# InterlinkLabs/e2e-tts

Measured on AMD Instinct MI355X. Metric: audio samples/sec (22.05 kHz, batch-32 per GPU, FastSpeech2 + HiFi-GAN inference, ids on host -> int16 PCM on host), higher is better.
Workload: dtype f32; 1 GPU; B=32/GPU fixed-length L=128 phonemes x 6 frames = T=768 frames (196608 samples, 8.92 s) per utterance; default model_config (6+6 FFT blocks H=384, HiFi-GAN V1), random-init weights; ids of tests/golden/bench_b32.npz (reference-pinned); global_batch=32, parallelism=utterance-sharded x1

## Files before the change

e2e_tts_amd/csrc/resblock_pair.hip:

```cpp
#include <algorithm>
#include <type_traits>

#include "kernels.h"

namespace e2etts {

typedef float f32x16 __attribute__((ext_vector_type(16)));
typedef __bf16 bf16x8 __attribute__((ext_vector_type(8)));
typedef __bf16 bf16x2 __attribute__((ext_vector_type(2)));

namespace {

constexpr int LDK = 36;
constexpr int MAX_HALO1 = 64;
constexpr size_t PAIR_MAX_LDS = 160 * 1024;

__device__ __forceinline__ unsigned pack_bf16(float a, float b) {
  const bf16x2 r = {(__bf16)a, (__bf16)b};
  return __builtin_bit_cast(unsigned, r);
}
__device__ __forceinline__ void split4(const float4 v, uint2& hi, uint2& lo) {
  hi.x = pack_bf16(v.x, v.y);
  hi.y = pack_bf16(v.z, v.w);
  const float hx = __builtin_bit_cast(float, hi.x << 16), hy = __builtin_bit_cast(float, hi.x & 0xffff0000u);
  const float hz = __builtin_bit_cast(float, hi.y << 16), hw = __builtin_bit_cast(float, hi.y & 0xffff0000u);
  lo.x = pack_bf16(v.x - hx, v.y - hy);
  lo.y = pack_bf16(v.z - hz, v.w - hw);
}

template <int BMI, int C, int WM, int WN>
constexpr int pair_threads() { return 64 * (BMI / WM) * (C / WN); }

template <int BMI, int C, int WM, int WN, int MODE, bool ACCUM>
__global__ __launch_bounds__((pair_threads<BMI, C, WM, WN>()), C == 32 ? 3 : 2) void resblock_pair_kernel(const PairParams p, const RowMap rm) {
  constexpr bool X3 = MODE != 0;
  constexpr bool SPLIT = MODE == 1;
  constexpr int KS = X3 ? 2 : 4;
  constexpr int NCH = C / 32;
  constexpr int NWN = C / WN;
  constexpr int MT = WM / 32, NT = WN / 32;
  constexpr int NWAVE = (BMI / WM) * NWN;
  static_assert(NWAVE == 4 || NWAVE == 8, "4 or 8 wavefronts per workgroup");
  constexpr int SROWS = NWAVE * 8;
  constexpr int AROWS = (BMI + MAX_HALO1 + SROWS - 1) / SROWS;

  extern __shared__ __attribute__((aligned(16))) float smem[];
  const int KW = p.KW, dil = p.dil;
  const int halo1 = dil * (KW - 1), pad1 = halo1 / 2, pad2 = (KW - 1) / 2;
  const int BMO = BMI - (KW - 1);
  const int irows = BMI + KW - 1;

  const int tid = threadIdx.x;
  const int lane = tid & 63, wave = __builtin_amdgcn_readfirstlane(tid >> 6);
  const int wm = wave / NWN, wn = wave % NWN;
  const int li = lane & 31, lh = lane >> 5;
  const int lrow = tid >> 3, lc4 = (tid & 7) * 4;

  int b, xb;
  if (rm.n > 0) {
    if (!rowmap_find(rm, (int)blockIdx.x, b, xb)) return;
  } else {
    b = blockIdx.y;
    xb = blockIdx.x;
  }
  const int t_act = p.act_rows ? min(p.act_rows[b], p.T) : p.T;
  const int mtiles = (t_act + BMO - 1) / BMO;
  const int eighth = (mtiles + 7) >> 3;
  const int tile = (xb & 7) * eighth + (xb >> 3);
  if ((xb >> 3) >= eighth || tile >= mtiles) return;

  const float* x_b = p.x + (long long)b * p.x_bs;
  float* out_b = p.out + (long long)b * p.out_bs;
  const __amdgpu_buffer_rsrc_t x_rsrc =
      __builtin_amdgcn_make_buffer_rsrc(const_cast<float*>(x_b), 0, (int)((long long)p.T * C * 4), 0x00020000);
  const int frag_words = NCH * KW * NCH * 1024;
  const __amdgpu_buffer_rsrc_t wf_rsrc =
      __builtin_amdgcn_make_buffer_rsrc(const_cast<float*>(p.wfrag), 0, 2 * frag_words * 4, 0x00020000);

  f32x16 acc[MT][NT];
#pragma unroll
  for (int m = 0; m < MT; ++m)
#pragma unroll
    for (int n = 0; n < NT; ++n)
#pragma unroll
      for (int r = 0; r < 16; ++r) acc[m][n][r] = 0.f;

  float4 areg[AROWS];
  bool aok[AROWS];
  const int srows = BMI + halo1;
  auto load_a = [&](int tile, int chunk) {
    const int x0 = tile * BMO - pad2 - pad1;
#pragma unroll
    for (int i = 0; i < AROWS; ++i) {
      const int r = lrow + i * SROWS;
      const int g = x0 + r;
      aok[i] = r < srows && g >= 0 && g < p.T;
      const int gc = min(max(g, 0), p.T - 1);
      areg[i] = __builtin_bit_cast(
          float4, __builtin_amdgcn_raw_buffer_load_b128(x_rsrc, (gc * C + lc4) * 4, chunk * 128, 0));
    }
  };
  auto store_a = [&]() {
#pragma unroll
    for (int i = 0; i < AROWS; ++i) {
      const int r = lrow + i * SROWS;
      if (r < srows) {
        float4 v = aok[i] ? areg[i] : make_float4(0.f, 0.f, 0.f, 0.f);
        v.x = fmaxf(v.x, v.x * p.slope); v.y = fmaxf(v.y, v.y * p.slope);
        v.z = fmaxf(v.z, v.z * p.slope); v.w = fmaxf(v.w, v.w * p.slope);
        if constexpr (X3) {
          uint2 hi, lo;
          split4(v, hi, lo);
          uint2* row = reinterpret_cast<uint2*>(smem + r * LDK);
          row[lc4 >> 2] = hi;
          row[8 + (lc4 >> 2)] = lo;
        } else {
          *reinterpret_cast<float4*>(smem + r * LDK + lc4) = v;
        }
      }
    }
  };

  constexpr bool DEEP = C == 32;
  float4 bfr[DEEP ? 2 : 1][KS][NT][SPLIT ? 2 : 1];
  auto load_frag_n = [&](auto par, int conv, int chunk, int j, int ks, int n) {
    constexpr int P = decltype(par)::value;
#pragma unroll
    for (int hl = 0; hl < (SPLIT ? 2 : 1); ++hl) {
      const int nt = wn * NT + n;
      const int piece = X3 ? ks * 2 + hl : ks;
      const int soff = (conv * frag_words + (((((nt * KW + j) * NCH + chunk) * 4) + piece) << 8)) * 4;
      bfr[P][ks][n][hl] = __builtin_bit_cast(float4, __builtin_amdgcn_raw_buffer_load_b128(wf_rsrc, lane * 16, soff, 0));
    }
  };
  auto load_frag = [&](int conv, int chunk, int j, int ks) {
#pragma unroll
    for (int n = 0; n < NT; ++n) load_frag_n(std::integral_constant<int, 0>{}, conv, chunk, j, ks, n);
  };
  auto mma_tap = [&](auto par, const float* a_base, int nconv, int nchunk, int nj) {
    constexpr int P = decltype(par)::value;
    if constexpr (DEEP) {
#pragma unroll
      for (int ks = 0; ks < KS; ++ks)
#pragma unroll
        for (int n = 0; n < NT; ++n) load_frag_n(std::integral_constant<int, 1 - P>{}, nconv, nchunk, nj, ks, n);
      __builtin_amdgcn_sched_barrier(0);
    }
#pragma unroll
    for (int ks = 0; ks < KS; ++ks) {
      if constexpr (X3) {
        bf16x8 ah[MT], al[MT];
#pragma unroll
        for (int m = 0; m < MT; ++m) {
          ah[m] = __builtin_bit_cast(bf16x8, *reinterpret_cast<const float4*>(a_base + m * 32 * LDK + ks * 8));
          if constexpr (SPLIT) al[m] = __builtin_bit_cast(bf16x8, *reinterpret_cast<const float4*>(a_base + m * 32 * LDK + 16 + ks * 8));
        }
#pragma unroll
        for (int n = 0; n < NT; ++n) {
#pragma unroll
          for (int m = 0; m < MT; ++m) {
            const bf16x8 bh = __builtin_bit_cast(bf16x8, bfr[P][ks][n][0]);
            if constexpr (SPLIT) {
              const bf16x8 bl = __builtin_bit_cast(bf16x8, bfr[P][ks][n][1]);
              acc[m][n] = __builtin_amdgcn_mfma_f32_32x32x16_bf16(bh, al[m], acc[m][n], 0, 0, 0);
              acc[m][n] = __builtin_amdgcn_mfma_f32_32x32x16_bf16(bl, ah[m], acc[m][n], 0, 0, 0);
            }
            acc[m][n] = __builtin_amdgcn_mfma_f32_32x32x16_bf16(bh, ah[m], acc[m][n], 0, 0, 0);
          }
          if constexpr (!DEEP) {
            __builtin_amdgcn_sched_barrier(0);
            load_frag_n(std::integral_constant<int, 0>{}, nconv, nchunk, nj, ks, n);
            __builtin_amdgcn_sched_barrier(0);
          }
        }
      } else {
        float4 af[MT];
#pragma unroll
        for (int m = 0; m < MT; ++m) af[m] = *reinterpret_cast<const float4*>(a_base + m * 32 * LDK + ks * 8);
#pragma unroll
        for (int n = 0; n < NT; ++n) {
          const float4 bf = bfr[P][ks][n][0];
#pragma unroll
          for (int m = 0; m < MT; ++m) {
            acc[m][n] = __builtin_amdgcn_mfma_f32_32x32x2f32(bf.x, af[m].x, acc[m][n], 0, 0, 0);
            acc[m][n] = __builtin_amdgcn_mfma_f32_32x32x2f32(bf.y, af[m].y, acc[m][n], 0, 0, 0);
            acc[m][n] = __builtin_amdgcn_mfma_f32_32x32x2f32(bf.z, af[m].z, acc[m][n], 0, 0, 0);
            acc[m][n] = __builtin_amdgcn_mfma_f32_32x32x2f32(bf.w, af[m].w, acc[m][n], 0, 0, 0);
          }
          if constexpr (!DEEP) {
            __builtin_amdgcn_sched_barrier(0);
            load_frag_n(std::integral_constant<int, 0>{}, nconv, nchunk, nj, ks, n);
            __builtin_amdgcn_sched_barrier(0);
          }
        }
      }
    }
  };
  auto run_taps = [&](auto par0, const float* a0, int row_step, int conv, int c, int nconv_end, int nchunk_end) {
    constexpr int P0 = DEEP ? decltype(par0)::value : 0;
    constexpr int P1 = DEEP ? 1 - P0 : 0;
    int j = 0;
    for (; j + 2 < KW; j += 2) {
      mma_tap(std::integral_constant<int, P0>{}, a0 + j * row_step, conv, c, j + 1);
      mma_tap(std::integral_constant<int, P1>{}, a0 + (j + 1) * row_step, conv, c, j + 2);
    }
    mma_tap(std::integral_constant<int, P0>{}, a0 + j * row_step, nconv_end, nchunk_end, 0);
  };

  auto epilogue1 = [&](int tile) {
    const int i0 = tile * BMO - pad2;
#pragma unroll
    for (int n = 0; n < NT; ++n) {
      const int chunk = wn * NT + n;
      float4 bq[4];
#pragma unroll
      for (int q = 0; q < 4; ++q) bq[q] = *reinterpret_cast<const float4*>(p.b1 + wn * WN + n * 32 + 8 * q + 4 * lh);
#pragma unroll
      for (int m = 0; m < MT; ++m) {
        const int row = wm * WM + m * 32 + li;
        const int g = i0 + row;
        const bool ok = g >= 0 && g < p.T;
        float* dst = smem + (chunk * irows + row) * LDK + 2 * lh;
#pragma unroll
        for (int q = 0; q < 4; ++q) {
          float v[4] = {acc[m][n][4 * q] + bq[q].x, acc[m][n][4 * q + 1] + bq[q].y, acc[m][n][4 * q + 2] + bq[q].z, acc[m][n][4 * q + 3] + bq[q].w};
#pragma unroll
          for (int i = 0; i < 4; ++i) {
            v[i] = fmaxf(v[i], v[i] * p.slope);
            v[i] = ok ? v[i] : 0.f;
            acc[m][n][4 * q + i] = 0.f;
          }
          if constexpr (!X3) {
            *reinterpret_cast<float4*>(smem + (chunk * irows + row) * LDK + 8 * q + 4 * lh) = make_float4(v[0], v[1], v[2], v[3]);
            continue;
          }
          uint2 hi;
          hi.x = pack_bf16(v[0], v[1]);
          hi.y = pack_bf16(v[2], v[3]);
          *reinterpret_cast<uint2*>(dst + 4 * q) = hi;
          if constexpr (SPLIT) {
            const float h0 = __builtin_bit_cast(float, hi.x << 16), h1 = __builtin_bit_cast(float, hi.x & 0xffff0000u);
            const float h2 = __builtin_bit_cast(float, hi.y << 16), h3 = __builtin_bit_cast(float, hi.y & 0xffff0000u);
            uint2 lo;
            lo.x = pack_bf16(v[0] - h0, v[1] - h1);
            lo.y = pack_bf16(v[2] - h2, v[3] - h3);
            *reinterpret_cast<uint2*>(dst + 16 + 4 * q) = lo;
          }
        }
      }
    }
  };

  constexpr int ELD = WN + 4;
  static_assert(NWAVE * 32 * ELD <= NCH * BMI * LDK, "epilogue patches must fit in the region (>= the intermediate: NCH x (BMI + KW - 1) rows)");
  constexpr int LPR = WN / 4, RPP = 64 / LPR, PASSES = 32 / RPP;
  const int prow = lane / LPR, pc4 = (lane % LPR) * 4;
  const int ecol = wn * WN + pc4;
  const float4 bias2 = *reinterpret_cast<const float4*>(p.b2 + ecol);
  auto epilogue2 = [&](int tile) {
    const int o0 = tile * BMO;
    const int t_end = min(o0 + BMO, p.T);
    float* patch = smem + wave * (32 * ELD);
#pragma unroll
    for (int m = 0; m < MT; ++m) {
      const int tb = o0 + wm * WM + m * 32;
      float4 resv[PASSES];
#pragma unroll
      for (int ps = 0; ps < PASSES; ++ps) {
        const int t = min(tb + ps * RPP + prow, p.T - 1);
        resv[ps] = *reinterpret_cast<const float4*>(x_b + (long long)t * C + ecol);
      }
      float4 accv[PASSES];
      if constexpr (ACCUM) {
#pragma unroll
        for (int ps = 0; ps < PASSES; ++ps) {
          const int t = min(tb + ps * RPP + prow, p.T - 1);
          accv[ps] = *reinterpret_cast<const float4*>(out_b + (long long)t * C + ecol);
        }
      }
#pragma unroll
      for (int n = 0; n < NT; ++n)
#pragma unroll
        for (int q = 0; q < 4; ++q)
          *reinterpret_cast<float4*>(patch + li * ELD + n * 32 + 8 * q + 4 * lh) =
              make_float4(acc[m][n][4 * q], acc[m][n][4 * q + 1], acc[m][n][4 * q + 2], acc[m][n][4 * q + 3]);
#pragma unroll
      for (int ps = 0; ps < PASSES; ++ps) {
        const int row = ps * RPP + prow;
        const int t = tb + row;
        float4 v = *reinterpret_cast<const float4*>(patch + row * ELD + pc4);
        v.x += bias2.x; v.y += bias2.y; v.z += bias2.z; v.w += bias2.w;
        const float4 rv = resv[ps];
        v.x += rv.x; v.y += rv.y; v.z += rv.z; v.w += rv.w;
        if constexpr (ACCUM) {
          const float4 ov = accv[ps];
          v.x += ov.x; v.y += ov.y; v.z += ov.z; v.w += ov.w;
          if (p.out_div != 1.0f) {
            v.x = v.x / p.out_div; v.y = v.y / p.out_div; v.z = v.z / p.out_div; v.w = v.w / p.out_div;
          }
        }
        if (t < t_end && wm * WM + m * 32 + row < BMO) {
          typedef float f32x4_t __attribute__((ext_vector_type(4)));
          const f32x4_t nv = {v.x, v.y, v.z, v.w};
          __builtin_nontemporal_store(nv, reinterpret_cast<f32x4_t*>(out_b + (long long)t * C + ecol));
        }
      }
    }
  };

  load_a(tile, 0);
  store_a();
#pragma unroll
  for (int ks = 0; ks < KS; ++ks) load_frag(0, 0, 0, ks);
  __builtin_amdgcn_s_waitcnt(0x0F70);

  for (int c = 0; c < NCH; ++c) {
    if (c + 1 < NCH) load_a(tile, c + 1);
    __syncthreads();
    const bool lastc = c + 1 == NCH;
    run_taps(std::integral_constant<int, 0>{}, smem + (wm * WM + li) * LDK + lh * 4, dil * LDK, 0, c, lastc ? 1 : 0, lastc ? 0 : c + 1);
    if (c + 1 < NCH) {
      __syncthreads();
      store_a();
    }
  }
  __syncthreads();
  epilogue1(tile);
  __syncthreads();
  for (int c = 0; c < NCH; ++c) {
    const bool lastc = c + 1 == NCH;
    run_taps(std::integral_constant<int, 1>{}, smem + (c * irows + wm * WM + li) * LDK + lh * 4, LDK, 1, c, 1, lastc ? 0 : c + 1);
  }
  __syncthreads();
  epilogue2(tile);
}

template <int BMI, int C, int WM, int WN, int MODE>
const char* launch_pair_cfg(const PairParams& p, hipStream_t s) {
  const int halo1 = p.dil * (p.KW - 1);
  const int BMO = BMI - (p.KW - 1);
  const size_t words = (size_t)std::max((BMI + halo1) * LDK, (C / 32) * (BMI + p.KW - 1) * LDK);
  const size_t lds = words * sizeof(float);
  if (lds > PAIR_MAX_LDS) return "resblock_pair: LDS region exceeds the CU's 160 KiB";
  const int mtiles = (p.T + BMO - 1) / BMO;
  dim3 grid((mtiles + 7) / 8 * 8, p.B);
  RowMap rm;
  if (p.act_rows && p.act_rows_host && p.B <= ROWMAP_MAX) {
    rm.n = p.B;
    rm.identity();
    rm.cum[0] = 0;
    for (int b = 0; b < p.B; ++b) {
      const int mt = (std::min(std::max(p.act_rows_host[b], 0), p.T) + BMO - 1) / BMO;
      rm.cum[b + 1] = rm.cum[b] + (mt + 7) / 8 * 8;
    }
    if (rm.cum[p.B] == 0) return nullptr;
    grid = dim3(rm.cum[p.B]);
  }
  constexpr int NTHR = pair_threads<BMI, C, WM, WN>();
  if (p.accumulate)
    hipLaunchKernelGGL((resblock_pair_kernel<BMI, C, WM, WN, MODE, true>), grid, dim3(NTHR), lds, s, p, rm);
  else
    hipLaunchKernelGGL((resblock_pair_kernel<BMI, C, WM, WN, MODE, false>), grid, dim3(NTHR), lds, s, p, rm);
  return hipGetLastError() == hipSuccess ? nullptr : "resblock_pair: launch failed";
}

template <int BMI, int C, int WM, int WN>
const char* launch_pair_mode(const PairParams& p, hipStream_t s) {
  static bool attr_done = false;
  if (!attr_done) {
    const int cap = C == 256 ? (int)PAIR_MAX_LDS : 80 * 1024;
    (void)hipFuncSetAttribute(reinterpret_cast<const void*>(&resblock_pair_kernel<BMI, C, WM, WN, 0, true>), hipFuncAttributeMaxDynamicSharedMemorySize, cap);
    (void)hipFuncSetAttribute(reinterpret_cast<const void*>(&resblock_pair_kernel<BMI, C, WM, WN, 0, false>), hipFuncAttributeMaxDynamicSharedMemorySize, cap);
    (void)hipFuncSetAttribute(reinterpret_cast<const void*>(&resblock_pair_kernel<BMI, C, WM, WN, 1, true>), hipFuncAttributeMaxDynamicSharedMemorySize, cap);
    (void)hipFuncSetAttribute(reinterpret_cast<const void*>(&resblock_pair_kernel<BMI, C, WM, WN, 1, false>), hipFuncAttributeMaxDynamicSharedMemorySize, cap);
    (void)hipFuncSetAttribute(reinterpret_cast<const void*>(&resblock_pair_kernel<BMI, C, WM, WN, 2, true>), hipFuncAttributeMaxDynamicSharedMemorySize, cap);
    (void)hipFuncSetAttribute(reinterpret_cast<const void*>(&resblock_pair_kernel<BMI, C, WM, WN, 2, false>), hipFuncAttributeMaxDynamicSharedMemorySize, cap);
    attr_done = true;
  }
  if (p.mode == 0) return launch_pair_cfg<BMI, C, WM, WN, 0>(p, s);
  return p.mode == 1 ? launch_pair_cfg<BMI, C, WM, WN, 1>(p, s) : launch_pair_cfg<BMI, C, WM, WN, 2>(p, s);
}

}

bool resblock_pair_supported(int C, int KW, int dil) {
  if (!((C == 32 || C == 64 || C == 128 || C == 256) && (KW & 1) && KW >= 3 && KW <= 15 && dil >= 1 && dil * (KW - 1) <= MAX_HALO1)) return false;
  return C != 256 || (size_t)(C / 32) * (128 + KW - 1) * LDK * 4 <= PAIR_MAX_LDS;
}

double resblock_pair_flops(const PairParams& p) { return 2.0 * 2.0 * p.B * (double)p.T * p.act_frac * p.C * p.KW * p.C; }

double resblock_pair_bytes(const PairParams& p) {
  return 4.0 * ((double)p.B * p.T * p.act_frac * p.C * (2.0 + (p.accumulate ? 1 : 0)) + 2.0 * p.C * p.KW * p.C);
}

const char* launch_resblock_pair(const PairParams& p, hipStream_t s) {
  if (!p.x || !p.wfrag || !p.b1 || !p.b2 || !p.out) return "resblock_pair: null pointer";
  if (p.B <= 0 || p.T <= 0) return "resblock_pair: bad dims";
  if (!resblock_pair_supported(p.C, p.KW, p.dil)) return "resblock_pair: unsupported channels / kernel / dilation";
  if (p.mode < 0 || p.mode > 2) return "resblock_pair: mode must be 0 (fp32), 1 (bf16x3) or 2 (bf16)";
  if (p.slope < 0.f || p.slope > 1.f) return "resblock_pair: slope must lie in [0, 1]";
  if (p.out_div != 1.0f && !p.accumulate) return "resblock_pair: out_div needs accumulate";
  if ((((uintptr_t)p.x | (uintptr_t)p.out | (uintptr_t)p.wfrag | (uintptr_t)p.b1 | (uintptr_t)p.b2) & 15) || (p.x_bs & 3) || (p.out_bs & 3))
    return "resblock_pair: pointers must be 16-byte aligned";
  if ((long long)p.T * p.C * 4 >= (1LL << 31)) return "resblock_pair: one utterance must stay below 2 GiB (32-bit buffer offsets)";
  if (p.x == p.out) return "resblock_pair: in-place is not possible (tiles read their neighbours' rows)";
  if (p.C == 32) return launch_pair_mode<256, 32, 64, 32>(p, s);
  if (p.C == 64) return launch_pair_mode<256, 64, 64, 64>(p, s);
  if (p.C == 256) return launch_pair_mode<128, 256, 64, 64>(p, s);
  return launch_pair_mode<128, 128, 64, 64>(p, s);
}

}
```

Measured before the change: 48.77 million audio samples/s.

## Double-buffer input slabs, prefetch A fragments, and share epilogue patch in bf16x3 resblock pair

```diff
diff --git a/e2e_tts_amd/csrc/resblock_pair.hip b/e2e_tts_amd/csrc/resblock_pair.hip
--- a/e2e_tts_amd/csrc/resblock_pair.hip
+++ b/e2e_tts_amd/csrc/resblock_pair.hip
@@ -1,4 +1,5 @@
 #include <algorithm>
+#include <cstdlib>
 #include <type_traits>
 
 #include "kernels.h"
@@ -31,10 +32,17 @@
 template <int BMI, int C, int WM, int WN>
 constexpr int pair_threads() { return 64 * (BMI / WM) * (C / WN); }
 
-template <int BMI, int C, int WM, int WN, int MODE, bool ACCUM>
+constexpr int PAIR_DBUF = 1, PAIR_AHEAD = 2;
+#define PAIR_INLINE __attribute__((always_inline))
+
+template <int BMI, int C, int WM, int WN, int MODE, bool ACCUM, int OPT = 0>
 __global__ __launch_bounds__((pair_threads<BMI, C, WM, WN>()), C == 32 ? 3 : 2) void resblock_pair_kernel(const PairParams p, const RowMap rm) {
   constexpr bool X3 = MODE != 0;
   constexpr bool SPLIT = MODE == 1;
+  constexpr bool DBUF = (OPT & PAIR_DBUF) != 0, AHEAD = (OPT & PAIR_AHEAD) != 0;
+  static_assert(OPT == 0 || SPLIT, "the options belong to the bf16x3 mode");
+  constexpr int SLAB1 = (BMI + MAX_HALO1) * LDK;
+  static_assert(!DBUF || (C >= 64 && 2 * SLAB1 <= (C / 32) * BMI * LDK), "two x slabs must fit in the region (>= the intermediate)");
   constexpr int KS = X3 ? 2 : 4;
   constexpr int NCH = C / 32;
   constexpr int NWN = C / WN;
@@ -207,6 +215,81 @@
     mma_tap(std::integral_constant<int, P0>{}, a0 + j * row_step, nconv_end, nchunk_end, 0);
   };
 
+  bf16x8 xh[AHEAD ? 2 : 1][MT], xl[AHEAD ? 2 : 1][MT];
+  auto read_x = [&](int set, const float* a_base, int ks) PAIR_INLINE {
+#pragma unroll
+    for (int m = 0; m < MT; ++m) {
+      xh[set][m] = __builtin_bit_cast(bf16x8, *reinterpret_cast<const float4*>(a_base + m * 32 * LDK + ks * 8));
+      xl[set][m] = __builtin_bit_cast(bf16x8, *reinterpret_cast<const float4*>(a_base + m * 32 * LDK + 16 + ks * 8));
+    }
+  };
+  static_assert(!DBUF || AROWS * SROWS == BMI + MAX_HALO1, "the staged rows fill the slab's allotment exactly");
+  auto load_a_nc = [&](int tile, int chunk) PAIR_INLINE {
+    const int x0 = tile * BMO - pad2 - pad1;
+#pragma unroll
+    for (int i = 0; i < AROWS; ++i)
+      areg[i] = __builtin_bit_cast(float4, __builtin_amdgcn_raw_buffer_load_b128(x_rsrc, ((x0 + lrow + i * SROWS) * C + lc4) * 4, chunk * 128, 0));
+  };
+  auto store_a_part = [&](int part, int slab) PAIR_INLINE {
+#pragma unroll
+    for (int i = 0; i < AROWS; ++i) {
+      const int r = lrow + i * SROWS;
+      if (i * 4 / AROWS == part) {
+        float4 v = areg[i];
+        v.x = fmaxf(v.x, v.x * p.slope); v.y = fmaxf(v.y, v.y * p.slope);
+        v.z = fmaxf(v.z, v.z * p.slope); v.w = fmaxf(v.w, v.w * p.slope);
+        uint2 hi, lo;
+        split4(v, hi, lo);
+        uint2* row = reinterpret_cast<uint2*>(smem + slab + r * LDK);
+        row[lc4 >> 2] = hi;
+        row[8 + (lc4 >> 2)] = lo;
+      }
+    }
+  };
+  auto mma_tap_opt = [&](auto stage, auto has_next, const float* a_base, int row_step, int slab, int nconv, int nchunk, int nj) PAIR_INLINE {
+    constexpr int STAGE = decltype(stage)::value;
+#pragma unroll
+    for (int ks = 0; ks < KS; ++ks) {
+      const int set = AHEAD ? ks : 0;
+      if constexpr (!AHEAD) {
+        read_x(0, a_base, ks);
+      } else {
+        if (ks == 0) read_x(1, a_base, 1);
+        else if (decltype(has_next)::value) read_x(0, a_base + row_step, 0);
+        __builtin_amdgcn_sched_barrier(0);
+      }
+#pragma unroll
+      for (int n = 0; n < NT; ++n) {
+        const bf16x8 bh = __builtin_bit_cast(bf16x8, bfr[0][ks][n][0]);
+        const bf16x8 bl = __builtin_bit_cast(bf16x8, bfr[0][ks][n][1]);
+#pragma unroll
+        for (int m = 0; m < MT; ++m) {
+          acc[m][n] = __builtin_amdgcn_mfma_f32_32x32x16_bf16(bh, xl[set][m], acc[m][n], 0, 0, 0);
+          acc[m][n] = __builtin_amdgcn_mfma_f32_32x32x16_bf16(bl, xh[set][m], acc[m][n], 0, 0, 0);
+          acc[m][n] = __builtin_amdgcn_mfma_f32_32x32x16_bf16(bh, xh[set][m], acc[m][n], 0, 0, 0);
+        }
+        if (STAGE >= 0 && n == 0) store_a_part(STAGE * 2 + ks, slab);
+        __builtin_amdgcn_sched_barrier(0);
+        load_frag_n(std::integral_constant<int, 0>{}, nconv, nchunk, nj, ks, n);
+        __builtin_amdgcn_sched_barrier(0);
+      }
+    }
+  };
+  auto run_taps_opt = [&](auto staged, const float* a0, int row_step, int slab, int conv, int c, int nconv_end, int nchunk_end) PAIR_INLINE {
+    constexpr bool ST = decltype(staged)::value;
+    using no = std::integral_constant<int, -1>;
+    using yes = std::true_type;
+    if constexpr (AHEAD) read_x(0, a0, 0);
+    int j = 0;
+    for (; j + 4 < KW; j += 2) {
+      mma_tap_opt(no{}, yes{}, a0 + j * row_step, row_step, slab, conv, c, j + 1);
+      mma_tap_opt(no{}, yes{}, a0 + (j + 1) * row_step, row_step, slab, conv, c, j + 2);
+    }
+    mma_tap_opt(no{}, yes{}, a0 + j * row_step, row_step, slab, conv, c, j + 1);
+    mma_tap_opt(std::integral_constant<int, ST ? 0 : -1>{}, yes{}, a0 + (j + 1) * row_step, row_step, slab, conv, c, j + 2);
+    mma_tap_opt(std::integral_constant<int, ST ? 1 : -1>{}, std::false_type{}, a0 + (j + 2) * row_step, row_step, slab, nconv_end, nchunk_end, 0);
+  };
+
   auto epilogue1 = [&](int tile) {
     const int i0 = tile * BMO - pad2;
 #pragma unroll
@@ -308,20 +391,88 @@
     }
   };
 
+  constexpr bool SHARED_PATCH = SPLIT && WN == 32 && NWN > 1;
+  constexpr int PLD = C + 4;
+  static_assert(!SHARED_PATCH || BMI * PLD <= NCH * BMI * LDK, "the shared patch must fit in the region (>= the intermediate: NCH x (BMI + KW - 1) rows)");
+  auto epilogue2_shared = [&](int tile) PAIR_INLINE {
+    constexpr int NTHR = 64 * NWAVE, CPR = C / 4, RPP = NTHR / CPR, NPASS = BMI / RPP, GRP = 4;
+    static_assert(NPASS % GRP == 0, "passes come in groups");
+    const int o0 = tile * BMO;
+    const int t_end = min(o0 + BMO, p.T);
+    const int prow = tid / CPR, col = (tid % CPR) * 4;
+    const float4 bias2 = *reinterpret_cast<const float4*>(p.b2 + col);
+    float4 resv[2][GRP], accv[2][GRP];
+    auto request = [&](int set, int g) PAIR_INLINE {
+#pragma unroll
+      for (int ps = 0; ps < GRP; ++ps) {
+        const int t = min(o0 + (g * GRP + ps) * RPP + prow, p.T - 1);
+        resv[set][ps] = *reinterpret_cast<const float4*>(x_b + (long long)t * C + col);
+        if constexpr (ACCUM) accv[set][ps] = *reinterpret_cast<const float4*>(out_b + (long long)t * C + col);
+      }
+    };
+    request(0, 0);
+#pragma unroll
+    for (int m = 0; m < MT; ++m)
+#pragma unroll
+      for (int n = 0; n < NT; ++n)
+#pragma unroll
+        for (int q = 0; q < 4; ++q)
+          *reinterpret_cast<float4*>(smem + (wm * WM + m * 32 + li) * PLD + wn * WN + n * 32 + 8 * q + 4 * lh) =
+              make_float4(acc[m][n][4 * q], acc[m][n][4 * q + 1], acc[m][n][4 * q + 2], acc[m][n][4 * q + 3]);
+    __syncthreads();
+#pragma unroll
+    for (int g = 0; g < NPASS / GRP; ++g) {
+      if (g + 1 < NPASS / GRP) request((g + 1) & 1, g + 1);
+#pragma unroll
+      for (int ps = 0; ps < GRP; ++ps) {
+        const int row = (g * GRP + ps) * RPP + prow;
+        const int t = o0 + row;
+        float4 v = *reinterpret_cast<const float4*>(smem + row * PLD + col);
+        v.x += bias2.x; v.y += bias2.y; v.z += bias2.z; v.w += bias2.w;
+        const float4 rv = resv[g & 1][ps];
+        v.x += rv.x; v.y += rv.y; v.z += rv.z; v.w += rv.w;
+        if constexpr (ACCUM) {
+          const float4 ov = accv[g & 1][ps];
+          v.x += ov.x; v.y += ov.y; v.z += ov.z; v.w += ov.w;
+          if (p.out_div != 1.0f) {
+            v.x = v.x / p.out_div; v.y = v.y / p.out_div; v.z = v.z / p.out_div; v.w = v.w / p.out_div;
+          }
+        }
+        if (t < t_end && row < BMO) {
+          typedef float f32x4_t __attribute__((ext_vector_type(4)));
+          const f32x4_t nv = {v.x, v.y, v.z, v.w};
+          __builtin_nontemporal_store(nv, reinterpret_cast<f32x4_t*>(out_b + (long long)t * C + col));
+        }
+      }
+    }
+  };
+
   load_a(tile, 0);
   store_a();
 #pragma unroll
   for (int ks = 0; ks < KS; ++ks) load_frag(0, 0, 0, ks);
   __builtin_amdgcn_s_waitcnt(0x0F70);
 
-  for (int c = 0; c < NCH; ++c) {
-    if (c + 1 < NCH) load_a(tile, c + 1);
+  if constexpr (DBUF) {
+    const float* a1 = smem + (wm * WM + li) * LDK + lh * 4;
+    for (int c = 0; c + 1 < NCH; ++c) {
+      load_a_nc(tile, c + 1);
+      __syncthreads();
+      run_taps_opt(std::true_type{}, a1 + (c & 1) * SLAB1, dil * LDK, ((c + 1) & 1) * SLAB1, 0, c, 0, c + 1);
+    }
     __syncthreads();
-    const bool lastc = c + 1 == NCH;
-    run_taps(std::integral_constant<int, 0>{}, smem + (wm * WM + li) * LDK + lh * 4, dil * LDK, 0, c, lastc ? 1 : 0, lastc ? 0 : c + 1);
-    if (c + 1 < NCH) {
+    run_taps_opt(std::false_type{}, a1 + ((NCH - 1) & 1) * SLAB1, dil * LDK, 0, 0, NCH - 1, 1, 0);
+  } else {
+    for (int c = 0; c < NCH; ++c) {
+      if (c + 1 < NCH) load_a(tile, c + 1);
       __syncthreads();
-      store_a();
+      const bool lastc = c + 1 == NCH;
+      if constexpr (AHEAD) run_taps_opt(std::false_type{}, smem + (wm * WM + li) * LDK + lh * 4, dil * LDK, 0, 0, c, lastc ? 1 : 0, lastc ? 0 : c + 1);
+      else run_taps(std::integral_constant<int, 0>{}, smem + (wm * WM + li) * LDK + lh * 4, dil * LDK, 0, c, lastc ? 1 : 0, lastc ? 0 : c + 1);
+      if (c + 1 < NCH) {
+        __syncthreads();
+        store_a();
+      }
     }
   }
   __syncthreads();
@@ -329,13 +480,15 @@
   __syncthreads();
   for (int c = 0; c < NCH; ++c) {
     const bool lastc = c + 1 == NCH;
-    run_taps(std::integral_constant<int, 1>{}, smem + (c * irows + wm * WM + li) * LDK + lh * 4, LDK, 1, c, 1, lastc ? 0 : c + 1);
+    if constexpr (AHEAD) run_taps_opt(std::false_type{}, smem + (c * irows + wm * WM + li) * LDK + lh * 4, LDK, 0, 1, c, 1, lastc ? 0 : c + 1);
+    else run_taps(std::integral_constant<int, 1>{}, smem + (c * irows + wm * WM + li) * LDK + lh * 4, LDK, 1, c, 1, lastc ? 0 : c + 1);
   }
   __syncthreads();
-  epilogue2(tile);
-}
-
-template <int BMI, int C, int WM, int WN, int MODE>
+  if constexpr (SHARED_PATCH) epilogue2_shared(tile);
+  else epilogue2(tile);
+}
+
+template <int BMI, int C, int WM, int WN, int MODE, int OPT = 0>
 const char* launch_pair_cfg(const PairParams& p, hipStream_t s) {
   const int halo1 = p.dil * (p.KW - 1);
   const int BMO = BMI - (p.KW - 1);
@@ -357,28 +510,45 @@
     grid = dim3(rm.cum[p.B]);
   }
   constexpr int NTHR = pair_threads<BMI, C, WM, WN>();
-  if (p.accumulate)
-    hipLaunchKernelGGL((resblock_pair_kernel<BMI, C, WM, WN, MODE, true>), grid, dim3(NTHR), lds, s, p, rm);
-  else
-    hipLaunchKernelGGL((resblock_pair_kernel<BMI, C, WM, WN, MODE, false>), grid, dim3(NTHR), lds, s, p, rm);
-  return hipGetLastError() == hipSuccess ? nullptr : "resblock_pair: launch failed";
-}
-
-template <int BMI, int C, int WM, int WN>
-const char* launch_pair_mode(const PairParams& p, hipStream_t s) {
   static bool attr_done = false;
   if (!attr_done) {
     const int cap = C == 256 ? (int)PAIR_MAX_LDS : 80 * 1024;
-    (void)hipFuncSetAttribute(reinterpret_cast<const void*>(&resblock_pair_kernel<BMI, C, WM, WN, 0, true>), hipFuncAttributeMaxDynamicSharedMemorySize, cap);
-    (void)hipFuncSetAttribute(reinterpret_cast<const void*>(&resblock_pair_kernel<BMI, C, WM, WN, 0, false>), hipFuncAttributeMaxDynamicSharedMemorySize, cap);
-    (void)hipFuncSetAttribute(reinterpret_cast<const void*>(&resblock_pair_kernel<BMI, C, WM, WN, 1, true>), hipFuncAttributeMaxDynamicSharedMemorySize, cap);
-    (void)hipFuncSetAttribute(reinterpret_cast<const void*>(&resblock_pair_kernel<BMI, C, WM, WN, 1, false>), hipFuncAttributeMaxDynamicSharedMemorySize, cap);
-    (void)hipFuncSetAttribute(reinterpret_cast<const void*>(&resblock_pair_kernel<BMI, C, WM, WN, 2, true>), hipFuncAttributeMaxDynamicSharedMemorySize, cap);
-    (void)hipFuncSetAttribute(reinterpret_cast<const void*>(&resblock_pair_kernel<BMI, C, WM, WN, 2, false>), hipFuncAttributeMaxDynamicSharedMemorySize, cap);
+    (void)hipFuncSetAttribute(reinterpret_cast<const void*>(&resblock_pair_kernel<BMI, C, WM, WN, MODE, true, OPT>), hipFuncAttributeMaxDynamicSharedMemorySize, cap);
+    (void)hipFuncSetAttribute(reinterpret_cast<const void*>(&resblock_pair_kernel<BMI, C, WM, WN, MODE, false, OPT>), hipFuncAttributeMaxDynamicSharedMemorySize, cap);
     attr_done = true;
   }
+  if (p.accumulate)
+    hipLaunchKernelGGL((resblock_pair_kernel<BMI, C, WM, WN, MODE, true, OPT>), grid, dim3(NTHR), lds, s, p, rm);
+  else
+    hipLaunchKernelGGL((resblock_pair_kernel<BMI, C, WM, WN, MODE, false, OPT>), grid, dim3(NTHR), lds, s, p, rm);
+  return hipGetLastError() == hipSuccess ? nullptr : "resblock_pair: launch failed";
+}
+
+template <int BMI, int C, int WM, int WN, int OPT>
+const char* launch_pair_tile(const PairParams& p, hipStream_t s, bool wide) {
+  if constexpr (C == 256) {
+    if (wide) return launch_pair_cfg<BMI, C, 128, 32, 1, OPT>(p, s);
+  }
+  return launch_pair_cfg<BMI, C, WM, WN, 1, OPT>(p, s);
+}
+
+template <int BMI, int C, int WM, int WN>
+const char* launch_pair_x3(const PairParams& p, hipStream_t s, int off) {
+  const bool dbuf = !(off & 1), wide = !(off & 2), ahead = !(off & 4);
+  if (dbuf) return ahead ? launch_pair_tile<BMI, C, WM, WN, PAIR_DBUF | PAIR_AHEAD>(p, s, wide) : launch_pair_tile<BMI, C, WM, WN, PAIR_DBUF>(p, s, wide);
+  return ahead ? launch_pair_tile<BMI, C, WM, WN, PAIR_AHEAD>(p, s, wide) : launch_pair_tile<BMI, C, WM, WN, 0>(p, s, wide);
+}
+
+template <int BMI, int C, int WM, int WN>
+const char* launch_pair_mode(const PairParams& p, hipStream_t s) {
   if (p.mode == 0) return launch_pair_cfg<BMI, C, WM, WN, 0>(p, s);
-  return p.mode == 1 ? launch_pair_cfg<BMI, C, WM, WN, 1>(p, s) : launch_pair_cfg<BMI, C, WM, WN, 2>(p, s);
+  if (p.mode == 2) return launch_pair_cfg<BMI, C, WM, WN, 2>(p, s);
+  if constexpr (C >= 128) {
+    static const int off = getenv("E2ETTS_PAIR_X3_OFF") ? atoi(getenv("E2ETTS_PAIR_X3_OFF")) : 0;
+    return launch_pair_x3<BMI, C, WM, WN>(p, s, off);
+  } else {
+    return launch_pair_cfg<BMI, C, WM, WN, 1>(p, s);
+  }
 }
 
 }
```

After: 48.72 million audio samples/s. No clear change (-0.1%).
